# arloan/OpticalImageProcessor

Measured on AMD Instinct MI355X. Metric: Mpix/s end-to-end RRC+stitch on 30000x100000x4 strip; % HBM roofline, higher is better.
Workload: dtype u16 rasters; fp64 RRC/maps, f32 bicubic and FFT; 1 GPU; default action (--do-rrc4pan): PAN 30000x100000 + MSS 4x(7500x25000) per GPU; RRC + 5x10x4 inter-band phase correlations (16000x3000 FFT) + polyfit + bicubic align to 16UC4; width=30000, pan_lines_per_gpu=100000, parallelism=rowblock1, backend=rccl, inputs=resident in HBM

## Files before the change

include/oip_c.h:

```cpp
#ifndef OIP_C_H
#define OIP_C_H

#include <stddef.h>
#include <stdint.h>

#ifdef __cplusplus
extern "C" {
#endif

typedef struct oip_ctx oip_ctx;

typedef enum oip_status {
    OIP_OK = 0,
    OIP_E_INVALID = 1,
    OIP_E_RUNTIME = 2,
    OIP_E_IO = 3,
    OIP_E_DEVICE = 4,
    OIP_E_NOMEM = 5,
    OIP_E_UNSUPPORTED = 6
} oip_status;

#define OIP_PIXELS_PER_LINE      12288
#define OIP_MSS_BANDS            4
#define OIP_CORRELATION_LINES    16000
// ... 110 lines not shown

int oip_stt_correlate_windows(oip_ctx *ctx, const uint16_t *const *d_a, const size_t *pitch_a,
                              const uint16_t *const *d_b, const size_t *pitch_b, int n, int rows, int cols,
                              double *out);

int oip_interband_correlate(oip_ctx *ctx, const uint16_t *d_pan, long Lp, long prow0, long pn,
                            const uint16_t *d_planes, size_t plane_stride, long mrow0, long mn,
                            int W, int slices, int sections, int corr_lines, double *out);

int oip_interband_correlate_units(oip_ctx *ctx, const uint16_t *const *d_pan, const size_t *pan_pitch,
                                  const uint16_t *const *d_bands, const size_t *band_pitch, int n, int rows,
                                  int cols, double *out);

int oip_peak_prune_stats(oip_ctx *ctx, long long *tiles_searched, long long *tiles_total);

int oip_upsample_operator(int n, float *out);

int oip_stt_mean(const double *table, int sections, double threshold, double max_delta_y, double *dx,
                 double *dy, double *response, int *valid);

#define OIP_FIT_REFERENCE 0
#define OIP_FIT_LSTSQ     1
int oip_filter_and_fit(const double *shifts, int n, double threshold, int min_count,
                       double *cx_out, double *cy_out, char *err, int errlen);
int oip_filter_and_fit_mode(const double *shifts, int n, double threshold, int min_count, int fit_mode,
                            double *cx_out, double *cy_out, char *err, int errlen);
int oip_polyfit_reference(const double *x, const double *y, int n, int deg, double *coeffs);
int oip_polyfit(const double *x, const double *y, int n, int deg, double *coeffs);

int oip_remap_shift_bicubic_u16(oip_ctx *ctx, const uint16_t *d_src, long src_row0,
// ... 129 lines not shown
```

opticalimageprocessor_amd/capi.py:

```python
from __future__ import annotations

import ctypes as C
import os
import re
import subprocess

import numpy as np

_PKG = os.path.dirname(os.path.abspath(__file__))
_ROOT = os.path.dirname(_PKG)
_LIB = None

STATUS_NAMES = {0: "OK", 1: "INVALID", 2: "RUNTIME", 3: "IO", 4: "DEVICE", 5: "NOMEM", 6: "UNSUPPORTED"}
_STATUS_EXC = {1: ValueError, 2: RuntimeError, 3: OSError, 4: RuntimeError, 5: MemoryError, 6: NotImplementedError}


class OipError(RuntimeError):
    def __init__(self, status, msg):
        super().__init__("oip status %s: %s" % (STATUS_NAMES.get(status, status), msg))
        self.status = status


def library_path() -> str:
    return os.environ.get("OIP_LIBRARY") or os.path.join(_PKG, "lib", "liboipgpu.so")
# ... 60 lines not shown
    "oip_download_staged": ([_vp, _vp, _vp, _sz], _i),
    "oip_stage_wait": ([_vp, _l], _i),
    "oip_stage_sync": ([_vp], _i),
    "oip_stage_order_after_compute": ([_vp], _i),
    "oip_stage_threads": ([], _i),
    "oip_stage_stats": ([_vp, _dp, _i], _i),
    "oip_mss_split_rrc_u16": ([_vp, _vp, _vp, _sz, _i, _l, _vp], _i),
    "oip_phase_correlate_f32": ([_vp, _vp, _vp, _i, _i, _dp, _dp, _dp], _i),
    "oip_window_u16_to_f32": ([_vp, _vp, _sz, _l, _i, _i, _i, _vp], _i),
    "oip_resize_cubic_f32": ([_vp, _vp, _i, _i, _vp, _i, _i], _i),
    "oip_stt_correlate": ([_vp, _vp, _vp, _i, _l, _l, _l, _i, _i, _i, _i, _dp], _i),
    "oip_stt_correlate_windows": ([_vp, _vp, _vp, _vp, _vp, _i, _i, _i, _dp], _i),
    "oip_interband_correlate_units": ([_vp, _vp, _vp, _vp, _vp, _i, _i, _i, _dp], _i),
    "oip_interband_correlate": ([_vp, _vp, _l, _l, _l, _vp, _sz, _l, _l, _i, _i, _i, _i, _dp], _i),
    "oip_peak_prune_stats": ([_vp, C.POINTER(C.c_longlong), C.POINTER(C.c_longlong)], _i),
    "oip_filter_and_fit": ([_dp, _i, _d, _i, _dp, _dp, _cp, _i], _i),
    "oip_filter_and_fit_mode": ([_dp, _i, _d, _i, _i, _dp, _dp, _cp, _i], _i),
    "oip_polyfit": ([_dp, _dp, _i, _i, _dp], _i),
    "oip_polyfit_reference": ([_dp, _dp, _i, _i, _dp], _i),
    "oip_stt_mean": ([_dp, _i, _d, _d, _dp, _dp, _dp, C.POINTER(_i)], _i),
    "oip_upsample_operator": ([_i, C.POINTER(C.c_float)], _i),
    "oip_remap_shift_bicubic_u16": ([_vp, _vp, _l, _l, _vp, _l, _l, _i, _l, _d, _d, _i, _i], _i),
    "oip_remap_shift_bicubic_u16_f16acc": ([_vp, _vp, _l, _l, _vp, _l, _l, _i, _l, _d, _d, _i, _i], _i),
    "oip_remap_shift_bicubic_u16_window": ([_vp, _vp, _l, _l, _vp, _l, _i, _l, _l, _l, _i, _l, _d, _d, _i, _i, _i], _i),
    "oip_remap_shift_rrc_bicubic_u16_window": ([_vp, _vp, _l, _l, _vp, _vp, _l, _i, _l, _l, _l, _i, _l, _d, _d, _i, _i, _i], _i),
    "oip_remap_shift_src_range": ([_l, _l, _l, _d, _i, _lp, _lp], _i),
    "oip_align_mss_bicubic_u16x4": ([_vp, _vp, _sz, _l, _l, _vp, _l, _l, _i, _l, _dp, _dp, _i, _i, _i, _i, _i, _lp], _i),
    "oip_align_mss_src_range": ([_l, _l, _l, _dp, _i, _i, _i, _i, _i, _i, _lp, _lp], _i),
    "oip_stitch_rows_u16": ([_vp, _vp, _vp, _vp, _i, _l, _i], _i),
    "oip_seam_moments_u16": ([_vp, _vp, _vp, _i, _l, _i, _i, _i, _i, _vp], _i),
# ... 578 lines not shown
        n = len(pan_ptrs)
        out = np.zeros((n, 4, 3))
        if n == 0:
            return out
        pp = (C.c_void_p * n)(*[_ptr(p) for p in pan_ptrs])
        bp = (C.c_void_p * (4 * n))(*[_ptr(p) for u in band_ptrs for p in u])
        qp = (C.c_size_t * n)(*pan_pitch); qb = (C.c_size_t * n)(*band_pitch)
        self._ck(self.lib.oip_interband_correlate_units(self.h, pp, qp, bp, qb, n, rows, cols, out.ctypes.data_as(_dp)))
        return out

    def peak_prune_stats(self):
        s, t = C.c_longlong(0), C.c_longlong(0)
        self._ck(self.lib.oip_peak_prune_stats(self.h, C.byref(s), C.byref(t)))
        return s.value, t.value

    def remap_shift_bicubic_u16(self, src, dst, W, L, dx, dy, section_rows=30000, row_guard=32767,
                                src_row0=0, src_rows=None, out_row0=0, out_rows=None, f16acc=False):
        src_rows = L if src_rows is None else src_rows
        out_rows = L if out_rows is None else out_rows
        fn = self.lib.oip_remap_shift_bicubic_u16_f16acc if f16acc else self.lib.oip_remap_shift_bicubic_u16
        self._ck(fn(self.h, _ptr(src), src_row0, src_rows, _ptr(dst), out_row0, out_rows, W, L, dx, dy,
                    section_rows, row_guard))

    def remap_shift_bicubic_u16_window(self, src, dst, dst_pitch, dst_col0, dst_col_off, W, L, dx, dy, section_rows=30000,
                                       row_guard=32767, src_row0=0, src_rows=None, out_row0=0, out_rows=None, f16acc=False):
        src_rows = L if src_rows is None else src_rows
        out_rows = L if out_rows is None else out_rows
        self._ck(self.lib.oip_remap_shift_bicubic_u16_window(self.h, _ptr(src), src_row0, src_rows, _ptr(dst), dst_pitch, dst_col0,
                                                             dst_col_off, out_row0, out_rows, W, L, dx, dy, section_rows, row_guard,
                                                             1 if f16acc else 0))
# ... 80 lines not shown
```

opticalimageprocessor_amd/csrc/oip_internal.h:

```cpp
#pragma once

#include <hip/hip_runtime.h>

#include <cstdarg>
#include <cstdint>
#include <cstdio>
#include <cstring>
#include <string>
#include <vector>

#include "oip_c.h"

struct oip_prof_entry {
    std::string name;
    double total_ms = 0.0;
    long launches = 0;
};
struct oip_prof_pending {
    int entry;
    hipEvent_t e0, e1;
    bool own_e0;
};

struct oip_fft_state;
// ... 34 lines not shown

    void *d_small = nullptr;
    void *h_small = nullptr;
    size_t small_bytes = 0;

    void *d_work = nullptr;
    size_t work_bytes = 0;

    oip_stage_state *stage = nullptr;
    void *d_stage[2] = {nullptr, nullptr};
    size_t stage_bytes = 0;

    oip_fft_state *fft = nullptr;
    std::vector<OipResizeTab> resize_tabs;
    unsigned long long *d_prune_stats = nullptr;

    bool prof_on = false;
    std::string prof_filter;
    std::vector<oip_prof_entry> prof;
    std::vector<oip_prof_pending> prof_pending;
    hipEvent_t prof_chain = nullptr;
    const char *prof_tag = nullptr;
};

int oip_fail(oip_ctx *ctx, int code, const char *fmt, ...);
int oip_prof_begin(oip_ctx *ctx, const char *name);
void oip_prof_end(oip_ctx *ctx, int pending);
int oip_workspace(oip_ctx *ctx, size_t bytes, void **out);
int oip_small(oip_ctx *ctx, size_t bytes);
void oip_fft_destroy(oip_ctx *ctx);
// ... 66 lines not shown
```

opticalimageprocessor_amd/csrc/phasecorr.hip:

```cpp
#include "oip_corrgeom.h"
#include "oip_fft.h"
#include "oip_fft_dev.h"
#include "oip_internal.h"

#include <cfloat>
#include <cmath>

namespace {

constexpr int kBlock = 256;

__global__ __launch_bounds__(kBlock) void window_u16_to_f32_kernel(const uint16_t *__restrict__ img, size_t pitch,
                                                                   long row0, int col0, int rows, int cols,
                                                                   float *__restrict__ out)
{
    long i = (long)blockIdx.x * kBlock + threadIdx.x;
    const long n = (long)rows * cols;
    const long stride = (long)gridDim.x * kBlock;
    for (; i < n; i += stride) {
        long y = i / cols;
        int x = (int)(i - y * cols);
        out[i] = (float)img[(size_t)(row0 + y) * pitch + col0 + x];
    }
}
// ... 384 lines not shown
}

struct UpRowsJob {
    const float2 *zp;
    const float2 *zn;
    long zn_stride;
    int Pn;
    float2 *out[4];
    const float2 *xtab;
    int nout;
    const float2 *vtab;
    const uint2 *raw16;
    const int *ypos_s;
    int m;
    float *bound;
};

__device__ __forceinline__ float2 cmulj(float2 a, float2 b)
{
    oipfft::oip_v2f t, r;
    asm("v_pk_mul_f32 %0, %1, %2 op_sel_hi:[0,1]" : "=v"(t) : "v"(oipfft::to_v(a)), "v"(oipfft::to_v(b)));
    asm("v_pk_fma_f32 %0, %1, %2, %3 op_sel:[1,1,0] op_sel_hi:[1,0,1] neg_hi:[1,0,0]" : "=v"(r) : "v"(oipfft::to_v(a)), "v"(oipfft::to_v(b)), "v"(t));
    return oipfft::to_f2(r);
}
__device__ __forceinline__ float2 cfma(float2 a, float2 b, float2 acc)
{
    oipfft::oip_v2f t, r;
    asm("v_pk_fma_f32 %0, %1, %2, %3 op_sel_hi:[0,1,1]" : "=v"(t) : "v"(oipfft::to_v(a)), "v"(oipfft::to_v(b)), "v"(oipfft::to_v(acc)));
    asm("v_pk_fma_f32 %0, %1, %2, %3 op_sel:[1,1,0] op_sel_hi:[1,0,1] neg_lo:[1,0,0]" : "=v"(r) : "v"(oipfft::to_v(a)), "v"(oipfft::to_v(b)), "v"(t));
    return oipfft::to_f2(r);
// ... 5 lines not shown
    asm("v_pk_fma_f32 %0, %1, %2, %3 op_sel:[1,1,0] op_sel_hi:[1,0,1] neg_hi:[1,0,0]" : "=v"(r) : "v"(oipfft::to_v(a)), "v"(oipfft::to_v(b)), "v"(t));
    return oipfft::to_f2(r);
}

__device__ __forceinline__ float2 spec2_of(int part, float2 zk, float2 zm)
{
    if (part == 0) return make_float2(zk.x + zm.x, zk.y - zm.y);
    return make_float2(zk.y + zm.y, zm.x - zk.x);
}
__device__ __forceinline__ float2 sfma(float s, float2 v, float2 acc)
{
    OIP_FFT_FMA
    return make_float2(acc.x + s * v.x, acc.y + s * v.y);
}

template <int NT, bool VEXP>
__global__ __launch_bounds__(NT) void corr_rows_up_kernel(UpRowsJob fj, int M, int P, const int *__restrict__ ypos,
                                                          const float2 *__restrict__ twF, const float2 *__restrict__ twS)
{
    constexpr int F = 3000, S = F / 4;
    constexpr int TWF = oipfft::TwTable<F, 25, 15, 8>::value(), TWS = oipfft::TwTable<S, 25, 15, 2>::value();
    constexpr int NB = (F / 2 + 1 + NT - 1) / NT;
    __shared__ __align__(16) float2 buf[2 * 2 * F + 4 * 2 * S];
    __shared__ float2 tw[TWF], tws[TWS];
    __shared__ float2 edge[4][2][4];
    __shared__ float2 edgeA[2][2];
    __shared__ float2 edgeT[2][5];
    float2 *bufN = buf + 4 * F;
    float4 *buf4 = reinterpret_cast<float4 *>(buf), *buf4N = reinterpret_cast<float4 *>(bufN);
    const int half = M / 2;
    int ky = blockIdx.x;
// ... 184 lines not shown
            __syncthreads();
            asm volatile("" : "+v"(tid));
            oipfft::StagesAll<F, NT, 2, 1, 25, 15, 8>::run(buf, tw, tid);
#pragma unroll
            for (int o = 0; o < 2; ++o) {
#pragma unroll
                for (int it = 0; it < NIT2; ++it) line_pair_read_conj<F>(ya[o][it], yb[o][it], buf4, o * F, tid + it * NT);
            }
            __syncthreads();
        };
        auto store = [&](int o0) {
#pragma unroll
            for (int o = 0; o < 2; ++o) {
                float2 *out = fj.out[o0 + o];
#pragma unroll
                for (int it = 0; it < NIT2; ++it) line_pair_store<F>(out, s1 * P, s2 * P, pair, ya[o][it], yb[o][it], tid + it * NT);
            }
        };
        auto bound_add = [&](int o0) {
            int tb = tid;
            asm volatile("" : "+v"(tb));
#pragma unroll
            for (int o = 0; o < 2; ++o) {
#pragma unroll
                for (int it = 0; it < NIT2; ++it) {
                    const int q = tb + it * NT;
                    if (q < F / 2) {
                        const float4 a = ya[o][it], b = yb[o][it];
                        float2 s = make_float2(fabsf(a.x) + fabsf(a.y), fabsf(a.z) + fabsf(a.w));
                        if (pair) { s.x += fabsf(b.x) + fabsf(b.y); s.y += fabsf(b.z) + fabsf(b.w); }
                        float *bp = reinterpret_cast<float *>(brow + (unsigned)((o0 + o) * P + 2 * q) * 4u);
// ... 318 lines not shown
}

OipAxisDigits digits_of(const std::vector<int> &f, int L)
{
    OipAxisDigits d;
    d.n = (int)f.size();
    d.L = L;
    for (int i = 0; i < 4; ++i) d.f[i] = i < d.n ? f[i] : 1;
    return d;
}

inline size_t align_up(size_t v, size_t a) { return (v + a - 1) / a * a; }
inline bool smooth_len(long n) { for (int p : {2, 3, 5}) while (n % p == 0) n /= p; return n == 1; }

constexpr float kPruneMargin = 0x1p-8f;
constexpr int kSelThreads = 1024, kSelCols = 64, kSelParts = kSelThreads / kSelCols, kSelMaxTiles = 1024;
struct PruneWork {
    float *bound;
    int groups;
    float *bt;
    int *flags;
    int *count;
    int *tiles;
    int *ticket;
    int T, vshift;
};

__global__ __launch_bounds__(kSelThreads) void col_sel_first_kernel(PruneWork pw, int P, int N, int full)
{
    __shared__ float sPart[kSelParts][kSelCols];
    __shared__ float sBt[kSelMaxTiles];
    __shared__ int sbest;
    const int a = blockIdx.y, T = pw.T, V = 1 << pw.vshift;
    const int xl = threadIdx.x & (kSelCols - 1), j = threadIdx.x / kSelCols, x0 = blockIdx.x * kSelCols;
    {
        const int x = x0 + xl < N ? x0 + xl : N - 1;
        const float *p = pw.bound + (long)a * P + x;
        float s = 0.f;
#pragma unroll 8
        for (int g = j; g < pw.groups; g += kSelParts) s += p[(long)g * 4 * P];
        sPart[j][xl] = s;
// ... 28 lines not shown
        float bv = -1.f;
        int bi = 0;
        for (int t = threadIdx.x; t < T; t += 64)
            if (sBt[t] > bv) { bv = sBt[t]; bi = t; }
#pragma unroll
        for (int off = 32; off > 0; off >>= 1) {
            const float ov = __shfl_xor(bv, off, 64);
            const int oi = __shfl_xor(bi, off, 64);
            if (ov > bv || (ov == bv && oi < bi)) { bv = ov; bi = oi; }
        }
        if (threadIdx.x == 0) sbest = bi;
    }
    __syncthreads();
    const int tm = sbest, tp = tm ? tm - 1 : T - 1, tn = tm + 1 < T ? tm + 1 : 0;
    int *listA = pw.tiles + (long)(0 * 4 + a) * T, *listP = pw.tiles + (long)(1 * 4 + a) * T;
    for (int t = threadIdx.x; t < T; t += kSelThreads) {
        pw.flags[a * T + t] = full ? 3 : (t == tm ? 3 : (t == tp || t == tn ? 1 : 0));
        if (full) { listA[t] = t; listP[t] = t; }
    }
    if (threadIdx.x == 0) {
        int nA = T, nP = T;
        if (!full) {
            listP[0] = tm;
            nP = 1;
            nA = 0;
            listA[nA++] = tm;
            if (tp != tm) listA[nA++] = tp;
            if (tn != tm && tn != tp) listA[nA++] = tn;
        }
        pw.count[0 * 4 + a] = nA;
        pw.count[1 * 4 + a] = nP;
        pw.count[2 * 4 + a] = 0;
        pw.count[3 * 4 + a] = 0;
    }
}

__device__ __forceinline__ float peak_slot_value(unsigned long long packed)
{
    if (!packed) return -INFINITY;
    unsigned u = (unsigned)(packed >> 32);
    u = (u & 0x80000000u) ? (u & 0x7fffffffu) : ~u;
    return __uint_as_float(u);
}

__global__ __launch_bounds__(kPeakSlots) void col_sel_second_kernel(PruneWork pw, const unsigned long long *__restrict__ slots,
                                                                   unsigned long long *__restrict__ stats)
{
    constexpr int NW = kPeakSlots / 64;
    __shared__ unsigned long long sb[2][NW];
    __shared__ int sflag[kSelMaxTiles];
    __shared__ int nA, nP;
    const int a = blockIdx.x, T = pw.T;
    const unsigned long long *s = slots + (long)a * 2 * kPeakSlots;
    unsigned long long b0 = s[threadIdx.x], b1 = s[kPeakSlots + threadIdx.x];
#pragma unroll
    for (int off = 32; off > 0; off >>= 1) {
        const unsigned long long o0 = __shfl_xor(b0, off, 64), o1 = __shfl_xor(b1, off, 64);
        b0 = o0 > b0 ? o0 : b0;
        b1 = o1 > b1 ? o1 : b1;
    }
    if ((threadIdx.x & 63) == 0) { sb[0][threadIdx.x >> 6] = b0; sb[1][threadIdx.x >> 6] = b1; }
    if (threadIdx.x == 0) { nA = 0; nP = 0; }
    for (int t = threadIdx.x; t < T; t += kPeakSlots) sflag[t] = pw.flags[a * T + t];
    __syncthreads();
    b0 = sb[0][0]; b1 = sb[1][0];
    for (int w = 1; w < NW; ++w) { b0 = sb[0][w] > b0 ? sb[0][w] : b0; b1 = sb[1][w] > b1 ? sb[1][w] : b1; }
    const float mm = fminf(peak_slot_value(b0), peak_slot_value(b1));
    for (int t = threadIdx.x; t < T; t += kPeakSlots) {
        if (sflag[t] & 2) continue;
        const float bt = pw.bt[a * T + t];
        const bool skip = bt * (1.f + kPruneMargin) < mm && mm < INFINITY;
        if (!skip) sflag[t] |= 4;
    }
    __syncthreads();
    int *listA = pw.tiles + (long)(2 * 4 + a) * T, *listP = pw.tiles + (long)(3 * 4 + a) * T;
    for (int t = threadIdx.x; t < T; t += kPeakSlots) {
        if (!(sflag[t] & 4)) continue;
        listP[atomicAdd(&nP, 1)] = t;
        const int nb[3] = {t ? t - 1 : T - 1, t, t + 1 < T ? t + 1 : 0};
#pragma unroll
        for (int d = 0; d < 3; ++d)
            if (!(atomicOr(&sflag[nb[d]], 1) & 1)) listA[atomicAdd(&nA, 1)] = nb[d];
    }
    __syncthreads();
    if (threadIdx.x == 0) {
        pw.count[2 * 4 + a] = nA;
        pw.count[3 * 4 + a] = nP;
        atomicAdd(&stats[0], (unsigned long long)(pw.count[1 * 4 + a] + nP));
        atomicAdd(&stats[1], (unsigned long long)T);
    }
}

struct PcWork {
    PruneWork prune;
    float2 *z[5];
    float2 *y[4];
    float *fa;
    float *fb[8];
    float *fsmall;
    unsigned long long *slots;
};

int carve(oip_ctx *ctx, const OipFft2dPlan *pl, int rows, int cols, int small_elems, int nz, int ny, int nfb, PcWork *w, bool prune = false)
{
    const int M = pl->M;
    memset(&w->prune, 0, sizeof w->prune);
    size_t bbytes = 0, tbytes = 0;
    if (prune) {
        PruneWork &pw = w->prune;
        pw.groups = ctx->cu_count < M / 2 + 1 ? ctx->cu_count : M / 2 + 1;
        pw.T = pl->passes[0].lane_tiles;
        pw.vshift = pl->passes[0].vshift;
        bbytes = align_up(sizeof(float) * (size_t)pw.groups * 4 * pl->P, 256);
        if (oip_fft_col_list_ok(pl, 4) && (1 << pw.vshift) <= kSelCols && pw.T <= kSelMaxTiles)
            tbytes = align_up(sizeof(int) * ((size_t)(4 + 4 + 16) * pw.T + 16 + 4), 256);
    }
    const size_t zbytes = align_up(sizeof(float2) * (size_t)M * pl->P, 256);
    const size_t fbytes = align_up(sizeof(float) * (size_t)rows * cols, 256);
    const size_t sbytes = align_up(sizeof(float) * (size_t)(small_elems > 0 ? small_elems : 1), 256);
    const size_t pbytes = align_up(sizeof(unsigned long long) * 4 * 2 * kPeakSlots, 256);
    size_t total = zbytes * (nz + ny) + fbytes * (1 + nfb) + sbytes + pbytes + bbytes + tbytes;
    void *ws;
    int rc = oip_workspace(ctx, total, &ws);
    if (rc) return rc;
    char *p = (char *)ws;
    if (bbytes) { w->prune.bound = (float *)p; p += bbytes; }
    if (tbytes) {
        PruneWork &pw = w->prune;
        pw.bt = (float *)p;
        pw.flags = (int *)p + 4 * pw.T;
        pw.count = (int *)p + 8 * pw.T;
        pw.ticket = (int *)p + 8 * pw.T + 16;
        pw.tiles = (int *)p + 8 * pw.T + 16 + 4;
        p += tbytes;
    }
    for (int i = 0; i < 5; ++i) { w->z[i] = i < nz ? (float2 *)p : nullptr; if (i < nz) p += zbytes; }
    for (int i = 0; i < 4; ++i) { w->y[i] = i < ny ? (float2 *)p : nullptr; if (i < ny) p += zbytes; }
    w->fa = (float *)p; p += fbytes;
    for (int i = 0; i < 8; ++i) { w->fb[i] = i < nfb ? (float *)p : nullptr; if (i < nfb) p += fbytes; }
    w->fsmall = (float *)p; p += sbytes;
    w->slots = (unsigned long long *)p;
    ctx->prof_chain = nullptr;
    OIP_HIP(ctx, hipMemsetAsync(w->slots, 0, sizeof(unsigned long long) * 4 * 2 * kPeakSlots, ctx->stream));
    if (w->prune.ticket) OIP_HIP(ctx, hipMemsetAsync(w->prune.ticket, 0, sizeof(int) * 4, ctx->stream));
    return OIP_OK;
}

int launch_window(oip_ctx *ctx, const uint16_t *img, size_t pitch, long row0, int col0, int rows, int cols, float *out)
{
    long n = (long)rows * cols;
    long blocks = (n + kBlock - 1) / kBlock;
    long cap = (long)ctx->cu_count * 32;
    if (blocks > cap) blocks = cap;
    if (blocks < 1) blocks = 1;
    OipProfScope prof(ctx, "window_u16_to_f32_kernel");
    hipLaunchKernelGGL(window_u16_to_f32_kernel, dim3((unsigned)blocks), dim3(kBlock), 0, ctx->stream, img, pitch, row0,
                       col0, rows, cols, out);
    OIP_HIP(ctx, hipGetLastError());
    return OIP_OK;
// ... 374 lines not shown
        const int r = y < 2 ? y : (y >= m - 2 ? y - (m - 4) : -1);
        if (PAIRS) {
            const unsigned ux = *reinterpret_cast<const unsigned *>(bx + y * pitch), uy = *reinterpret_cast<const unsigned *>(by + y * pitch);
            *reinterpret_cast<float4 *>(z + (long)y * Pn + a * n + p) =
                make_float4((float)(ux & 0xffffu), (float)(uy & 0xffffu), (float)(ux >> 16), (float)(uy >> 16));
            if (r >= 0) *reinterpret_cast<uint2 *>(raw16 + ((long)r * 4 + a) * n + p) = make_uint2((ux & 0xffffu) | (uy << 16), (ux >> 16) | (uy & 0xffff0000u));
        } else {
            const unsigned ux = bx[y * pitch], uy = by[y * pitch];
            z[(long)y * Pn + a * n + p] = make_float2((float)ux, (float)uy);
            if (r >= 0) raw16[((long)r * 4 + a) * n + p] = ux | (uy << 16);
        }
    }
}

int correlate_units_up(oip_ctx *ctx, const OipFft2dPlan *pl, const UpPath &up, const PcWork &w, RealSrc aA, RealSrc aB, const RealSrc *v ,
                       const IbUnit *const *units, int nunits, int rows, int cols, int band_rows, int band_cols, double *d_resA, double *d_resB)
{
    int rc;
    if ((rc = forward_packed(ctx, pl, w.z[0], aA, nunits > 1 ? aB : src_none(), rows, cols, true))) return rc;
    const int narr = 2 * nunits;
    long zn_stride;
    int Pn;
    const int *ypos_s = nullptr;
    unsigned *raw = nullptr;
    if (up.vtab) {
        Pn = up.small->P;
        zn_stride = band_cols;
        raw = reinterpret_cast<unsigned *>(w.z[1] + (long)up.small->M * Pn);
        BandPackJob bj;
        for (int a = 0; a < 4; ++a) {
            const IbUnit *u = units[(a < narr ? a : 0) / 2];
// ... 33 lines not shown
    memset(&fj, 0, sizeof fj);
    fj.zp = w.z[0];
    fj.zn = w.z[1];
    fj.zn_stride = zn_stride;
    fj.Pn = Pn;
    for (int o = 0; o < 4; ++o) fj.out[o] = w.y[o];
    fj.xtab = up.xtab;
    fj.nout = narr;
    fj.vtab = up.vtab;
    fj.raw16 = reinterpret_cast<const uint2 *>(raw);
    fj.ypos_s = ypos_s;
    fj.m = band_rows;
    fj.bound = w.prune.bound;
    if (!fj.bound) return oip_fail(ctx, OIP_E_RUNTIME, "correlate_units_up: no storage for the column bounds");
    OIP_HIP(ctx, hipMemsetAsync(fj.bound, 0, sizeof(float) * (size_t)w.prune.groups * 4 * pl->P, ctx->stream));
    {
        OipProfScope prof(ctx, "corr_rows_up_kernel");
        const long grid = w.prune.groups;
        const dim3 g((unsigned)grid);
        if (up.vtab)
            hipLaunchKernelGGL((corr_rows_up_kernel<512, true>), g, dim3(512), 0, ctx->stream, fj, pl->M, pl->P, pl->d_ypos, twF, twS);
        else
            hipLaunchKernelGGL((corr_rows_up_kernel<512, false>), g, dim3(512), 0, ctx->stream, fj, pl->M, pl->P, pl->d_ypos, twF, twS);
        OIP_HIP(ctx, hipGetLastError());
    }
    double *res[4];
    for (int o = 0; o < narr; ++o) res[o] = (o < 2 ? d_resA : d_resB) + 6 * (o & 1);
    const PruneWork &pw = w.prune;
    if (!pw.tiles) {
        for (int o = 0; o < narr; ++o)
            if ((rc = inverse_to_slots(ctx, pl, w, w.y[o], true, o))) return rc;
        return peak_windows(ctx, pl, w, w.y, res, narr, 2);
    }
    const char *pe = getenv("OIP_PEAK_PRUNE");
    const int full = pe && atoi(pe) == 0 ? 1 : 0;
    if (!ctx->d_prune_stats) {
        OIP_HIP(ctx, hipMalloc((void **)&ctx->d_prune_stats, 2 * sizeof(unsigned long long)));
        OIP_HIP(ctx, hipMemsetAsync(ctx->d_prune_stats, 0, 2 * sizeof(unsigned long long), ctx->stream));
    }
    {
        OipProfScope prof(ctx, "col_sel_first_kernel");
        hipLaunchKernelGGL(col_sel_first_kernel, dim3((pl->N + kSelCols - 1) / kSelCols, narr), dim3(kSelThreads), 0, ctx->stream, pw, pl->P, pl->N, full);
        OIP_HIP(ctx, hipGetLastError());
    }
    OipColList cl;
    memset(&cl, 0, sizeof cl);
    for (int o = 0; o < 4; ++o) cl.data[o] = w.y[o < narr ? o : 0];
    cl.stride = pw.T;
    cl.narr = narr;
    cl.slots = w.slots;
// ... 67 lines not shown
        if (grid > pl->M / 2 + 1) grid = pl->M / 2 + 1;
        if (N != 1250) return oip_fail(ctx, OIP_E_RUNTIME, "correlate_units_vup: no row stage for %d-point rows", N);
        for (int u = 0; u < nunits; ++u)
            hipLaunchKernelGGL((corr_rows_v_kernel<1250, 512, 5, 5, 5, 5, 2>), dim3((unsigned)grid), dim3(512), 0, ctx->stream, fj, 2 * u, u, pl->M, pl->P,
                               pl->d_ypos, twF);
        OIP_HIP(ctx, hipGetLastError());
    }
    double *res[4];
    for (int o = 0; o < narr; ++o) {
        res[o] = (o < 2 ? d_resA : d_resB) + 6 * (o & 1);
        if ((rc = inverse_to_slots(ctx, pl, w, w.y[o], true, o))) return rc;
    }
    return peak_windows(ctx, pl, w, w.y, res, narr, 2);
}

int fetch_results(oip_ctx *ctx, int count, double *host_out)
{
    ctx->prof_chain = nullptr;
    OIP_HIP(ctx, hipMemcpyAsync(ctx->h_small, ctx->d_small, sizeof(double) * count, hipMemcpyDeviceToHost, ctx->stream));
    OIP_HIP(ctx, hipStreamSynchronize(ctx->stream));
    memcpy(host_out, ctx->h_small, sizeof(double) * count);
    return OIP_OK;
}

}

extern "C" int oip_window_u16_to_f32(oip_ctx *ctx, const uint16_t *d_img, size_t pitch, long row0, int col0, int rows,
                                     int cols, float *d_out)
{
    OIP_CHECK_CTX(ctx);
    if (!d_img || !d_out || rows <= 0 || cols <= 0 || row0 < 0 || col0 < 0 || (size_t)(col0 + cols) > pitch)
        return oip_fail(ctx, OIP_E_INVALID, "oip_window_u16_to_f32: bad argument");
    return launch_window(ctx, d_img, pitch, row0, col0, rows, cols, d_out);
}

extern "C" int oip_resize_cubic_f32(oip_ctx *ctx, const float *d_src, int sw, int sh, float *d_dst, int dw, int dh)
// ... 114 lines not shown
        }
        const char *ev = getenv("OIP_SPECTRAL_V");
        if (!up.xtab && !(ev && atoi(ev) == 0) && want > 0 && rows == 4 * band_rows && cols == 4 * band_cols && M == rows && N == 1250 &&
            (cols & 1) == 0 && row_stage(pl) && optimal_dft_size(band_rows) == band_rows && band_rows >= 8 && smooth_len(4 * N)) {
            if ((rc = upsample_spectrum_tables(ctx, tab, 1, &up.vtab))) return rc;
            if (up.vtab) {
                if ((rc = oip_fft2d_plan(ctx, band_rows, 4 * N, &up.small))) return rc;
                up.vonly = (long)up.small->M * up.small->P <= (long)pl->M * pl->P;
                if (!up.vonly) up.vtab = nullptr;
            }
        }
    }
    PcWork w;
    const bool spectral = up.xtab || up.vonly;
    if ((rc = carve(ctx, pl, rows, band_cols, up.vonly ? 32 * N : 0, spectral ? 2 : 5, spectral ? 4 : 2, 8, &w, up.xtab != nullptr))) return rc;
    if ((rc = oip_small(ctx, sizeof(double) * 12 * (size_t)(n > 0 ? n : 1)))) return rc;
    double *d_res = (double *)ctx->d_small;
    auto upsample = [&](const IbUnit *const *uns, int nun, float *const *fb, RealSrc *out) -> int {
        const uint16_t *srcs[kVBatch];
        long pitches[kVBatch];
        for (int u = 0; u < nun; ++u)
            for (int b = 0; b < OIP_MSS_BANDS; ++b) {
                srcs[4 * u + b] = uns[u]->band[b];
                pitches[4 * u + b] = uns[u]->band_pitch;
                out[4 * u + b] = src_v(fb[4 * u + b]);
            }
        return launch_resize_v<uint16_t>(ctx, srcs, fb, 4 * nun, pitches, band_cols, band_rows, cols, rows, &tab);
    };
    int k = 0;
    RealSrc sAB[8];
    for (; k + 1 < n; k += 2) {
        const IbUnit &A = units[k], &B = units[k + 1];
        const IbUnit *two[2] = {&A, &B};
        if (up.vonly) {
            if ((rc = correlate_units_vup(ctx, pl, up, w, tab, src_u16(A.pan, A.pan_pitch), src_u16(B.pan, B.pan_pitch), two, 2, rows, cols, band_rows,
                                          band_cols, d_res + 12 * k, d_res + 12 * (k + 1)))) return rc;
            continue;
        }
        if (!up.vtab && (rc = upsample(two, 2, w.fb, sAB))) return rc;
        if (up.xtab) {
            if ((rc = correlate_units_up(ctx, pl, up, w, src_u16(A.pan, A.pan_pitch), src_u16(B.pan, B.pan_pitch), sAB, two, 2, rows, cols, band_rows,
                                         band_cols, d_res + 12 * k, d_res + 12 * (k + 1)))) return rc;
            continue;
        }
        const HTaps vt{band_cols, tab->d_xofs, tab->d_alpha, tab->x4h};
        if ((rc = correlate_two_units(ctx, pl, w, src_u16(A.pan, A.pan_pitch), sAB, src_u16(B.pan, B.pan_pitch), sAB + 4, rows, cols,
                                      d_res + 12 * k, d_res + 12 * (k + 1), &vt))) return rc;
    }
    if (k < n) {
        const IbUnit &A = units[k];
        const IbUnit *one[1] = {&A};
        if (up.vonly) {
            if ((rc = correlate_units_vup(ctx, pl, up, w, tab, src_u16(A.pan, A.pan_pitch), src_none(), one, 1, rows, cols, band_rows, band_cols,
                                          d_res + 12 * k, nullptr))) return rc;
        } else {
        if (!up.vtab && (rc = upsample(one, 1, w.fb, sAB))) return rc;
        if (up.xtab) {
            if ((rc = correlate_units_up(ctx, pl, up, w, src_u16(A.pan, A.pan_pitch), src_none(), sAB, one, 1, rows, cols, band_rows, band_cols,
                                         d_res + 12 * k, nullptr))) return rc;
        } else {
            const HTaps vt{band_cols, tab->d_xofs, tab->d_alpha, tab->x4h};
            if ((rc = correlate_one_to_four(ctx, pl, w, src_u16(A.pan, A.pan_pitch), sAB, rows, cols, d_res + 12 * k, &vt))) return rc;
        }
        }
    }
    if (n > 0 && (rc = fetch_results(ctx, 12 * n, host_out))) return rc;
    return OIP_OK;
}

extern "C" int oip_peak_prune_stats(oip_ctx *ctx, long long *tiles_searched, long long *tiles_total)
{
    OIP_CHECK_CTX(ctx);
    unsigned long long *h = nullptr;
    if (ctx->d_prune_stats) {
        int rc = oip_small(ctx, 2 * sizeof(unsigned long long));
        if (rc) return rc;
        h = (unsigned long long *)ctx->h_small;
        OIP_HIP(ctx, hipMemcpyAsync(h, ctx->d_prune_stats, 2 * sizeof(unsigned long long), hipMemcpyDeviceToHost, ctx->stream));
        OIP_HIP(ctx, hipMemsetAsync(ctx->d_prune_stats, 0, 2 * sizeof(unsigned long long), ctx->stream));
        OIP_HIP(ctx, hipStreamSynchronize(ctx->stream));
    }
    if (tiles_searched) *tiles_searched = h ? (long long)h[0] : 0;
    if (tiles_total) *tiles_total = h ? (long long)h[1] : 0;
    return OIP_OK;
}

extern "C" int oip_interband_correlate_units(oip_ctx *ctx, const uint16_t *const *d_pan, const size_t *pan_pitch,
                                             const uint16_t *const *d_bands, const size_t *band_pitch, int n, int rows,
                                             int cols, double *out)
{
    OIP_CHECK_CTX(ctx);
    if (n < 0 || (n > 0 && (!d_pan || !pan_pitch || !d_bands || !band_pitch || !out)) || rows <= 0 || cols <= 0)
        return oip_fail(ctx, OIP_E_INVALID, "oip_interband_correlate_units: bad argument");
    const int band_rows = rows / OIP_MSS_BANDS, band_cols = cols / OIP_MSS_BANDS;
    if (band_rows <= 0 || band_cols <= 0) return oip_fail(ctx, OIP_E_INVALID, "oip_interband_correlate_units: window too small");
    std::vector<IbUnit> units((size_t)n);
    for (int i = 0; i < n; ++i) {
        units[i].pan = d_pan[i];
// ... 43 lines not shown
```

Measured before the change: 83470 Mpix/s.

## Store only a window of correlation rows near zero shift, rerun on peak miss

The row-pass kernel of the upsampled inter-band correlation now writes only the spectral rows within a radius of tiles around the wrap-around origin. The peak-selection kernels flag a miss when a candidate tile or its neighbours fall outside the stored window. The host reads back the miss flags and reruns affected pairs with the full store. This cuts HBM writes for the correlation surface, at the cost of an extra host sync and possible reruns when shifts are large.

```diff
diff --git a/include/oip_c.h b/include/oip_c.h
--- a/include/oip_c.h
+++ b/include/oip_c.h
@@ -148,6 +148,9 @@
 
 int oip_peak_prune_stats(oip_ctx *ctx, long long *tiles_searched, long long *tiles_total);
 
+int oip_rows_window_stats(oip_ctx *ctx, long long *pairs, long long *pairs_rerun);
+int oip_rows_window_geometry(oip_ctx *ctx, int *tile_cols, int *tiles, int *radius);
+
 int oip_upsample_operator(int n, float *out);
 
 int oip_stt_mean(const double *table, int sections, double threshold, double max_delta_y, double *dx,
diff --git a/opticalimageprocessor_amd/capi.py b/opticalimageprocessor_amd/capi.py
--- a/opticalimageprocessor_amd/capi.py
+++ b/opticalimageprocessor_amd/capi.py
@@ -98,6 +98,8 @@
     "oip_interband_correlate_units": ([_vp, _vp, _vp, _vp, _vp, _i, _i, _i, _dp], _i),
     "oip_interband_correlate": ([_vp, _vp, _l, _l, _l, _vp, _sz, _l, _l, _i, _i, _i, _i, _dp], _i),
     "oip_peak_prune_stats": ([_vp, C.POINTER(C.c_longlong), C.POINTER(C.c_longlong)], _i),
+    "oip_rows_window_stats": ([_vp, C.POINTER(C.c_longlong), C.POINTER(C.c_longlong)], _i),
+    "oip_rows_window_geometry": ([_vp, C.POINTER(C.c_int), C.POINTER(C.c_int), C.POINTER(C.c_int)], _i),
     "oip_filter_and_fit": ([_dp, _i, _d, _i, _dp, _dp, _cp, _i], _i),
     "oip_filter_and_fit_mode": ([_dp, _i, _d, _i, _i, _dp, _dp, _cp, _i], _i),
     "oip_polyfit": ([_dp, _dp, _i, _i, _dp], _i),
@@ -706,6 +708,16 @@
         self._ck(self.lib.oip_peak_prune_stats(self.h, C.byref(s), C.byref(t)))
         return s.value, t.value
 
+    def rows_window_stats(self):
+        p, r = C.c_longlong(0), C.c_longlong(0)
+        self._ck(self.lib.oip_rows_window_stats(self.h, C.byref(p), C.byref(r)))
+        return p.value, r.value
+
+    def rows_window_geometry(self):
+        v, t, r = C.c_int(0), C.c_int(0), C.c_int(-1)
+        self._ck(self.lib.oip_rows_window_geometry(self.h, C.byref(v), C.byref(t), C.byref(r)))
+        return v.value, t.value, r.value
+
     def remap_shift_bicubic_u16(self, src, dst, W, L, dx, dy, section_rows=30000, row_guard=32767,
                                 src_row0=0, src_rows=None, out_row0=0, out_rows=None, f16acc=False):
         src_rows = L if src_rows is None else src_rows
diff --git a/opticalimageprocessor_amd/csrc/oip_internal.h b/opticalimageprocessor_amd/csrc/oip_internal.h
--- a/opticalimageprocessor_amd/csrc/oip_internal.h
+++ b/opticalimageprocessor_amd/csrc/oip_internal.h
@@ -72,6 +72,8 @@
     oip_fft_state *fft = nullptr;
     std::vector<OipResizeTab> resize_tabs;
     unsigned long long *d_prune_stats = nullptr;
+    long long rows_window_pairs = 0, rows_window_rerun = 0;
+    int rows_window[3] = {0, 0, -1};
 
     bool prof_on = false;
     std::string prof_filter;
diff --git a/opticalimageprocessor_amd/csrc/phasecorr.hip b/opticalimageprocessor_amd/csrc/phasecorr.hip
--- a/opticalimageprocessor_amd/csrc/phasecorr.hip
+++ b/opticalimageprocessor_amd/csrc/phasecorr.hip
@@ -422,6 +422,7 @@
     const int *ypos_s;
     int m;
     float *bound;
+    int win_hi, win_lo;
 };
 
 __device__ __forceinline__ float2 cmulj(float2 a, float2 b)
@@ -457,7 +458,7 @@
     return make_float2(acc.x + s * v.x, acc.y + s * v.y);
 }
 
-template <int NT, bool VEXP>
+template <int NT, bool VEXP, bool WIN>
 __global__ __launch_bounds__(NT) void corr_rows_up_kernel(UpRowsJob fj, int M, int P, const int *__restrict__ ypos,
                                                           const float2 *__restrict__ twF, const float2 *__restrict__ twS)
 {
@@ -672,7 +673,10 @@
             for (int o = 0; o < 2; ++o) {
                 float2 *out = fj.out[o0 + o];
 #pragma unroll
-                for (int it = 0; it < NIT2; ++it) line_pair_store<F>(out, s1 * P, s2 * P, pair, ya[o][it], yb[o][it], tid + it * NT);
+                for (int it = 0; it < NIT2; ++it) {
+                    const int q = tid + it * NT;
+                    if (!WIN || q < fj.win_hi || q >= fj.win_lo) line_pair_store<F>(out, s1 * P, s2 * P, pair, ya[o][it], yb[o][it], q);
+                }
             }
         };
         auto bound_add = [&](int o0) {
@@ -1021,6 +1025,7 @@
 inline bool smooth_len(long n) { for (int p : {2, 3, 5}) while (n % p == 0) n /= p; return n == 1; }
 
 constexpr float kPruneMargin = 0x1p-8f;
+constexpr int kRowsWindowTiles = 8;
 constexpr int kSelThreads = 1024, kSelCols = 64, kSelParts = kSelThreads / kSelCols, kSelMaxTiles = 1024;
 struct PruneWork {
     float *bound;
@@ -1031,7 +1036,11 @@
     int *tiles;
     int *ticket;
     int T, vshift;
+    int win_r;
+    int *miss;
 };
+inline bool rows_window_fits(const PruneWork &pw, int r) { return r >= 0 && pw.tiles && pw.vshift >= 1 && 2 * r + 1 < pw.T; }
+__device__ __forceinline__ bool tile_stored(const PruneWork &pw, int t) { return pw.win_r < 0 || t <= pw.win_r || t >= pw.T - pw.win_r; }
 
 __global__ __launch_bounds__(kSelThreads) void col_sel_first_kernel(PruneWork pw, int P, int N, int full)
 {
@@ -1090,13 +1099,17 @@
     __syncthreads();
     const int tm = sbest, tp = tm ? tm - 1 : T - 1, tn = tm + 1 < T ? tm + 1 : 0;
     int *listA = pw.tiles + (long)(0 * 4 + a) * T, *listP = pw.tiles + (long)(1 * 4 + a) * T;
+    const bool missed = !full && !(tile_stored(pw, tm) && tile_stored(pw, tp) && tile_stored(pw, tn));
     for (int t = threadIdx.x; t < T; t += kSelThreads) {
-        pw.flags[a * T + t] = full ? 3 : (t == tm ? 3 : (t == tp || t == tn ? 1 : 0));
+        pw.flags[a * T + t] = full ? 3 : (missed ? 0 : (t == tm ? 3 : (t == tp || t == tn ? 1 : 0)));
         if (full) { listA[t] = t; listP[t] = t; }
     }
     if (threadIdx.x == 0) {
         int nA = T, nP = T;
-        if (!full) {
+        if (missed) {
+            atomicExch(pw.miss, 1);
+            nA = nP = 0;
+        } else if (!full) {
             listP[0] = tm;
             nP = 1;
             nA = 0;
@@ -1125,7 +1138,7 @@
     constexpr int NW = kPeakSlots / 64;
     __shared__ unsigned long long sb[2][NW];
     __shared__ int sflag[kSelMaxTiles];
-    __shared__ int nA, nP;
+    __shared__ int nA, nP, smiss;
     const int a = blockIdx.x, T = pw.T;
     const unsigned long long *s = slots + (long)a * 2 * kPeakSlots;
     unsigned long long b0 = s[threadIdx.x], b1 = s[kPeakSlots + threadIdx.x];
@@ -1142,15 +1155,24 @@
     b0 = sb[0][0]; b1 = sb[1][0];
     for (int w = 1; w < NW; ++w) { b0 = sb[0][w] > b0 ? sb[0][w] : b0; b1 = sb[1][w] > b1 ? sb[1][w] : b1; }
     const float mm = fminf(peak_slot_value(b0), peak_slot_value(b1));
-    for (int t = threadIdx.x; t < T; t += kPeakSlots) {
+    if (threadIdx.x == 0) smiss = pw.win_r >= 0 ? atomicAdd(pw.miss, 0) : 0;
+    __syncthreads();
+    const bool dead = smiss != 0;
+    __syncthreads();
+    for (int t = threadIdx.x; t < T && !dead; t += kPeakSlots) {
         if (sflag[t] & 2) continue;
         const float bt = pw.bt[a * T + t];
         const bool skip = bt * (1.f + kPruneMargin) < mm && mm < INFINITY;
-        if (!skip) sflag[t] |= 4;
+        if (!skip) {
+            sflag[t] |= 4;
+            const int tp = t ? t - 1 : T - 1, tn = t + 1 < T ? t + 1 : 0;
+            if (!(tile_stored(pw, t) && tile_stored(pw, tp) && tile_stored(pw, tn))) smiss = 1;
+        }
     }
     __syncthreads();
+    const bool missed = smiss != 0;
     int *listA = pw.tiles + (long)(2 * 4 + a) * T, *listP = pw.tiles + (long)(3 * 4 + a) * T;
-    for (int t = threadIdx.x; t < T; t += kPeakSlots) {
+    for (int t = threadIdx.x; t < T && !missed; t += kPeakSlots) {
         if (!(sflag[t] & 4)) continue;
         listP[atomicAdd(&nP, 1)] = t;
         const int nb[3] = {t ? t - 1 : T - 1, t, t + 1 < T ? t + 1 : 0};
@@ -1162,8 +1184,18 @@
     if (threadIdx.x == 0) {
         pw.count[2 * 4 + a] = nA;
         pw.count[3 * 4 + a] = nP;
-        atomicAdd(&stats[0], (unsigned long long)(pw.count[1 * 4 + a] + nP));
-        atomicAdd(&stats[1], (unsigned long long)T);
+        if (missed && !dead) atomicExch(pw.miss, 1);
+        __threadfence();
+        if (atomicAdd(&pw.ticket[4], 1) == (int)gridDim.x - 1) {
+            __threadfence();
+            atomicExch(&pw.ticket[4], 0);
+            if (pw.win_r < 0 || atomicAdd(pw.miss, 0) == 0) {
+                unsigned long long searched = 0;
+                for (int o = 0; o < (int)gridDim.x; ++o) searched += (unsigned long long)(atomicAdd(&pw.count[1 * 4 + o], 0) + atomicAdd(&pw.count[3 * 4 + o], 0));
+                atomicAdd(&stats[0], searched);
+                atomicAdd(&stats[1], (unsigned long long)T * gridDim.x);
+            }
+        }
     }
 }
 
@@ -1181,6 +1213,7 @@
 {
     const int M = pl->M;
     memset(&w->prune, 0, sizeof w->prune);
+    w->prune.win_r = -1;
     size_t bbytes = 0, tbytes = 0;
     if (prune) {
         PruneWork &pw = w->prune;
@@ -1189,7 +1222,7 @@
         pw.vshift = pl->passes[0].vshift;
         bbytes = align_up(sizeof(float) * (size_t)pw.groups * 4 * pl->P, 256);
         if (oip_fft_col_list_ok(pl, 4) && (1 << pw.vshift) <= kSelCols && pw.T <= kSelMaxTiles)
-            tbytes = align_up(sizeof(int) * ((size_t)(4 + 4 + 16) * pw.T + 16 + 4), 256);
+            tbytes = align_up(sizeof(int) * ((size_t)(4 + 4 + 16) * pw.T + 16 + 8), 256);
     }
     const size_t zbytes = align_up(sizeof(float2) * (size_t)M * pl->P, 256);
     const size_t fbytes = align_up(sizeof(float) * (size_t)rows * cols, 256);
@@ -1207,7 +1240,7 @@
         pw.flags = (int *)p + 4 * pw.T;
         pw.count = (int *)p + 8 * pw.T;
         pw.ticket = (int *)p + 8 * pw.T + 16;
-        pw.tiles = (int *)p + 8 * pw.T + 16 + 4;
+        pw.tiles = (int *)p + 8 * pw.T + 16 + 8;
         p += tbytes;
     }
     for (int i = 0; i < 5; ++i) { w->z[i] = i < nz ? (float2 *)p : nullptr; if (i < nz) p += zbytes; }
@@ -1218,7 +1251,7 @@
     w->slots = (unsigned long long *)p;
     ctx->prof_chain = nullptr;
     OIP_HIP(ctx, hipMemsetAsync(w->slots, 0, sizeof(unsigned long long) * 4 * 2 * kPeakSlots, ctx->stream));
-    if (w->prune.ticket) OIP_HIP(ctx, hipMemsetAsync(w->prune.ticket, 0, sizeof(int) * 4, ctx->stream));
+    if (w->prune.ticket) OIP_HIP(ctx, hipMemsetAsync(w->prune.ticket, 0, sizeof(int) * 8, ctx->stream));
     return OIP_OK;
 }
 
@@ -1623,7 +1656,8 @@
 }
 
 int correlate_units_up(oip_ctx *ctx, const OipFft2dPlan *pl, const UpPath &up, const PcWork &w, RealSrc aA, RealSrc aB, const RealSrc *v ,
-                       const IbUnit *const *units, int nunits, int rows, int cols, int band_rows, int band_cols, double *d_resA, double *d_resB)
+                       const IbUnit *const *units, int nunits, int rows, int cols, int band_rows, int band_cols, double *d_resA, double *d_resB,
+                       int win_r = -1, int *d_miss = nullptr)
 {
     int rc;
     if ((rc = forward_packed(ctx, pl, w.z[0], aA, nunits > 1 ? aB : src_none(), rows, cols, true))) return rc;
@@ -1687,26 +1721,37 @@
     fj.bound = w.prune.bound;
     if (!fj.bound) return oip_fail(ctx, OIP_E_RUNTIME, "correlate_units_up: no storage for the column bounds");
     OIP_HIP(ctx, hipMemsetAsync(fj.bound, 0, sizeof(float) * (size_t)w.prune.groups * 4 * pl->P, ctx->stream));
+    PruneWork pw = w.prune;
+    const char *pe = getenv("OIP_PEAK_PRUNE");
+    const int full = pe && atoi(pe) == 0 ? 1 : 0;
+    if (full || !up.vtab || !rows_window_fits(pw, win_r) || !d_miss) win_r = -1;
+    pw.win_r = win_r;
+    pw.miss = d_miss;
+    if (win_r >= 0) {
+        fj.win_hi = ((win_r + 1) << pw.vshift) / 2;
+        fj.win_lo = ((pw.T - win_r) << pw.vshift) / 2;
+    }
+    {
+        const char *pz = getenv("OIP_ROWS_WINDOW_POISON");
+        if (pz && atoi(pz) > 0)
+            for (int o = 0; o < narr; ++o) OIP_HIP(ctx, hipMemsetAsync(w.y[o], 0xff, sizeof(float2) * (size_t)pl->M * pl->P, ctx->stream));
+    }
     {
         OipProfScope prof(ctx, "corr_rows_up_kernel");
         const long grid = w.prune.groups;
         const dim3 g((unsigned)grid);
-        if (up.vtab)
-            hipLaunchKernelGGL((corr_rows_up_kernel<512, true>), g, dim3(512), 0, ctx->stream, fj, pl->M, pl->P, pl->d_ypos, twF, twS);
-        else
-            hipLaunchKernelGGL((corr_rows_up_kernel<512, false>), g, dim3(512), 0, ctx->stream, fj, pl->M, pl->P, pl->d_ypos, twF, twS);
+        auto k = up.vtab ? (win_r >= 0 ? corr_rows_up_kernel<512, true, true> : corr_rows_up_kernel<512, true, false>)
+                         : corr_rows_up_kernel<512, false, false>;
+        hipLaunchKernelGGL(k, g, dim3(512), 0, ctx->stream, fj, pl->M, pl->P, pl->d_ypos, twF, twS);
         OIP_HIP(ctx, hipGetLastError());
     }
     double *res[4];
     for (int o = 0; o < narr; ++o) res[o] = (o < 2 ? d_resA : d_resB) + 6 * (o & 1);
-    const PruneWork &pw = w.prune;
     if (!pw.tiles) {
         for (int o = 0; o < narr; ++o)
             if ((rc = inverse_to_slots(ctx, pl, w, w.y[o], true, o))) return rc;
         return peak_windows(ctx, pl, w, w.y, res, narr, 2);
     }
-    const char *pe = getenv("OIP_PEAK_PRUNE");
-    const int full = pe && atoi(pe) == 0 ? 1 : 0;
     if (!ctx->d_prune_stats) {
         OIP_HIP(ctx, hipMalloc((void **)&ctx->d_prune_stats, 2 * sizeof(unsigned long long)));
         OIP_HIP(ctx, hipMemsetAsync(ctx->d_prune_stats, 0, 2 * sizeof(unsigned long long), ctx->stream));
@@ -1804,12 +1849,13 @@
     return peak_windows(ctx, pl, w, w.y, res, narr, 2);
 }
 
-int fetch_results(oip_ctx *ctx, int count, double *host_out)
+int fetch_results(oip_ctx *ctx, int count, double *host_out, int nflags = 0, int *flags_out = nullptr)
 {
     ctx->prof_chain = nullptr;
-    OIP_HIP(ctx, hipMemcpyAsync(ctx->h_small, ctx->d_small, sizeof(double) * count, hipMemcpyDeviceToHost, ctx->stream));
+    OIP_HIP(ctx, hipMemcpyAsync(ctx->h_small, ctx->d_small, sizeof(double) * count + sizeof(int) * nflags, hipMemcpyDeviceToHost, ctx->stream));
     OIP_HIP(ctx, hipStreamSynchronize(ctx->stream));
     memcpy(host_out, ctx->h_small, sizeof(double) * count);
+    if (nflags) memcpy(flags_out, (const char *)ctx->h_small + sizeof(double) * count, sizeof(int) * nflags);
     return OIP_OK;
 }
 
@@ -1954,8 +2000,21 @@
     PcWork w;
     const bool spectral = up.xtab || up.vonly;
     if ((rc = carve(ctx, pl, rows, band_cols, up.vonly ? 32 * N : 0, spectral ? 2 : 5, spectral ? 4 : 2, 8, &w, up.xtab != nullptr))) return rc;
-    if ((rc = oip_small(ctx, sizeof(double) * 12 * (size_t)(n > 0 ? n : 1)))) return rc;
+    int win_r = -1;
+    if (up.xtab && up.vtab) {
+        const char *e = getenv("OIP_ROWS_WINDOW");
+        win_r = e ? atoi(e) : kRowsWindowTiles;
+        const char *pe = getenv("OIP_PEAK_PRUNE");
+        win_r = win_r > 0 && !(pe && atoi(pe) == 0) && rows_window_fits(w.prune, win_r) ? win_r : -1;
+    }
+    ctx->rows_window[0] = w.prune.tiles ? 1 << w.prune.vshift : 0;
+    ctx->rows_window[1] = w.prune.tiles ? w.prune.T : 0;
+    ctx->rows_window[2] = win_r;
+    const int ngroups = (n + 1) / 2;
+    if ((rc = oip_small(ctx, sizeof(double) * 12 * (size_t)(n > 0 ? n : 1) + sizeof(int) * (size_t)(ngroups + 1)))) return rc;
     double *d_res = (double *)ctx->d_small;
+    int *d_miss = reinterpret_cast<int *>(d_res + 12 * (size_t)n);
+    if (win_r >= 0) OIP_HIP(ctx, hipMemsetAsync(d_miss, 0, sizeof(int) * ngroups, ctx->stream));
     auto upsample = [&](const IbUnit *const *uns, int nun, float *const *fb, RealSrc *out) -> int {
         const uint16_t *srcs[kVBatch];
         long pitches[kVBatch];
@@ -1967,42 +2026,48 @@
             }
         return launch_resize_v<uint16_t>(ctx, srcs, fb, 4 * nun, pitches, band_cols, band_rows, cols, rows, &tab);
     };
-    int k = 0;
     RealSrc sAB[8];
-    for (; k + 1 < n; k += 2) {
-        const IbUnit &A = units[k], &B = units[k + 1];
-        const IbUnit *two[2] = {&A, &B};
-        if (up.vonly) {
-            if ((rc = correlate_units_vup(ctx, pl, up, w, tab, src_u16(A.pan, A.pan_pitch), src_u16(B.pan, B.pan_pitch), two, 2, rows, cols, band_rows,
-                                          band_cols, d_res + 12 * k, d_res + 12 * (k + 1)))) return rc;
-            continue;
-        }
-        if (!up.vtab && (rc = upsample(two, 2, w.fb, sAB))) return rc;
-        if (up.xtab) {
-            if ((rc = correlate_units_up(ctx, pl, up, w, src_u16(A.pan, A.pan_pitch), src_u16(B.pan, B.pan_pitch), sAB, two, 2, rows, cols, band_rows,
-                                         band_cols, d_res + 12 * k, d_res + 12 * (k + 1)))) return rc;
-            continue;
-        }
-        const HTaps vt{band_cols, tab->d_xofs, tab->d_alpha, tab->x4h};
-        if ((rc = correlate_two_units(ctx, pl, w, src_u16(A.pan, A.pan_pitch), sAB, src_u16(B.pan, B.pan_pitch), sAB + 4, rows, cols,
-                                      d_res + 12 * k, d_res + 12 * (k + 1), &vt))) return rc;
-    }
-    if (k < n) {
+    auto run_group = [&](int k, int wr) -> int {
+        if (k + 1 < n) {
+            const IbUnit &A = units[k], &B = units[k + 1];
+            const IbUnit *two[2] = {&A, &B};
+            if (up.vonly)
+                return correlate_units_vup(ctx, pl, up, w, tab, src_u16(A.pan, A.pan_pitch), src_u16(B.pan, B.pan_pitch), two, 2, rows, cols, band_rows,
+                                           band_cols, d_res + 12 * k, d_res + 12 * (k + 1));
+            if (!up.vtab && (rc = upsample(two, 2, w.fb, sAB))) return rc;
+            if (up.xtab)
+                return correlate_units_up(ctx, pl, up, w, src_u16(A.pan, A.pan_pitch), src_u16(B.pan, B.pan_pitch), sAB, two, 2, rows, cols, band_rows,
+                                          band_cols, d_res + 12 * k, d_res + 12 * (k + 1), wr, d_miss + k / 2);
+            const HTaps vt{band_cols, tab->d_xofs, tab->d_alpha, tab->x4h};
+            return correlate_two_units(ctx, pl, w, src_u16(A.pan, A.pan_pitch), sAB, src_u16(B.pan, B.pan_pitch), sAB + 4, rows, cols,
+                                       d_res + 12 * k, d_res + 12 * (k + 1), &vt);
+        }
         const IbUnit &A = units[k];
         const IbUnit *one[1] = {&A};
-        if (up.vonly) {
-            if ((rc = correlate_units_vup(ctx, pl, up, w, tab, src_u16(A.pan, A.pan_pitch), src_none(), one, 1, rows, cols, band_rows, band_cols,
-                                          d_res + 12 * k, nullptr))) return rc;
-        } else {
+        if (up.vonly)
+            return correlate_units_vup(ctx, pl, up, w, tab, src_u16(A.pan, A.pan_pitch), src_none(), one, 1, rows, cols, band_rows, band_cols,
+                                       d_res + 12 * k, nullptr);
         if (!up.vtab && (rc = upsample(one, 1, w.fb, sAB))) return rc;
-        if (up.xtab) {
-            if ((rc = correlate_units_up(ctx, pl, up, w, src_u16(A.pan, A.pan_pitch), src_none(), sAB, one, 1, rows, cols, band_rows, band_cols,
-                                         d_res + 12 * k, nullptr))) return rc;
-        } else {
-            const HTaps vt{band_cols, tab->d_xofs, tab->d_alpha, tab->x4h};
-            if ((rc = correlate_one_to_four(ctx, pl, w, src_u16(A.pan, A.pan_pitch), sAB, rows, cols, d_res + 12 * k, &vt))) return rc;
-        }
-        }
+        if (up.xtab)
+            return correlate_units_up(ctx, pl, up, w, src_u16(A.pan, A.pan_pitch), src_none(), sAB, one, 1, rows, cols, band_rows, band_cols,
+                                      d_res + 12 * k, nullptr, wr, d_miss + k / 2);
+        const HTaps vt{band_cols, tab->d_xofs, tab->d_alpha, tab->x4h};
+        return correlate_one_to_four(ctx, pl, w, src_u16(A.pan, A.pan_pitch), sAB, rows, cols, d_res + 12 * k, &vt);
+    };
+    for (int k = 0; k < n; k += 2)
+        if ((rc = run_group(k, win_r))) return rc;
+    if (n > 0 && win_r >= 0) {
+        std::vector<int> miss((size_t)ngroups);
+        if ((rc = fetch_results(ctx, 12 * n, host_out, ngroups, miss.data()))) return rc;
+        int again = 0;
+        for (int g = 0; g < ngroups; ++g)
+            if (miss[g]) {
+                ++again;
+                if ((rc = run_group(2 * g, -1))) return rc;
+            }
+        ctx->rows_window_pairs += ngroups;
+        ctx->rows_window_rerun += again;
+        if (!again) return OIP_OK;
     }
     if (n > 0 && (rc = fetch_results(ctx, 12 * n, host_out))) return rc;
     return OIP_OK;
@@ -2022,6 +2087,24 @@
     }
     if (tiles_searched) *tiles_searched = h ? (long long)h[0] : 0;
     if (tiles_total) *tiles_total = h ? (long long)h[1] : 0;
+    return OIP_OK;
+}
+
+extern "C" int oip_rows_window_stats(oip_ctx *ctx, long long *pairs, long long *pairs_rerun)
+{
+    OIP_CHECK_CTX(ctx);
+    if (pairs) *pairs = ctx->rows_window_pairs;
+    if (pairs_rerun) *pairs_rerun = ctx->rows_window_rerun;
+    ctx->rows_window_pairs = ctx->rows_window_rerun = 0;
+    return OIP_OK;
+}
+
+extern "C" int oip_rows_window_geometry(oip_ctx *ctx, int *tile_cols, int *tiles, int *radius)
+{
+    OIP_CHECK_CTX(ctx);
+    if (tile_cols) *tile_cols = ctx->rows_window[0];
+    if (tiles) *tiles = ctx->rows_window[1];
+    if (radius) *radius = ctx->rows_window[2];
     return OIP_OK;
 }
 
```

After: 88040 Mpix/s, median of 6. 5.5% higher.
